# LJacksonPan/RaTrack

Hardware: AMD Instinct MI355X
Metric: radar frame-pairs/sec (backbone forward, eval) at B=64,N=256 per GPU (higher is better)
Workload: dtype f32 (2xfp16 split MFMA: three fp16 products per fp32 product, fp32 accumulate, power-of-two scales per matrix and position); 1 GPU; Track4D.backbone forward, B=64 frame-pairs x N=256 points per GPU, S=512 centroids, eval-mode BN, random-init weights, hipGraph=True, batches in flight=4; global_batch=64, parallelism=replicas x1 (no collective on the forward path)

## Files before the change

include/rtk_fused.h:

```cpp
#ifndef RTK_FUSED_H
#define RTK_FUSED_H

#include "rtk_pointnet2.h"

#ifdef __cplusplus
extern "C" {
#endif

#define RTK_MAX_SRC 4
#define RTK_MAX_LAYERS 4

typedef struct {
    const float *ptr;
    int pitch;
    int channels;
    int per_sample;
} rtk_src_t;

#define RTK_LAYER_SPLIT 0x100
typedef struct {
    const float *w_packed;
    const float *bias;
    int cin16, cout16;
    int act;
    float inv_scale;
} rtk_layer_t;

typedef struct {
    const float *known_feats;
    int pitch, channels, m;
    const int *idx;
    const float *dist2;
    const int *nuniq;
} rtk_interp_t;

RTK_EXPORT int rtk_pointwise_mlp(int rows, int rows_per_sample, const rtk_interp_t *interp, int nsrc,
                                 const rtk_src_t *srcs, const float *sample_bias, int nlayers,
                                 const rtk_layer_t *layers, float *out, int out_pitch, int out_channels,
                                 int out_channel_major, const int *row_nuniq, float *colmax, rtk_stream_t stream);

RTK_EXPORT int rtk_pointwise_mlp_tap(int rows, int rows_per_sample, const rtk_interp_t *interp, const rtk_layer_t *layer, float *out,
                                     int out_pitch, float *colmax, const rtk_layer_t *proj, int frame_split, float *proj_out,
                                     int proj_pitch, rtk_stream_t stream);

RTK_EXPORT int rtk_sa_scale(int samples, int n, int npoint, int nsample, const float *xyz,
                            const float *new_xyz, const int *idx, const float *q, int q_pitch, int c1_16,
                            const float *w1xyz_packed, int nlayers, const rtk_layer_t *layers, float *out,
                            int out_pitch, int out_offset, const int *src_nuniq, const int *dst_nuniq,
                            rtk_stream_t stream);

RTK_EXPORT int rtk_cost_volume(int samples, int n1, int n2, const float *xyz1, const float *xyz2,
                               const int64_t *knn_idx, const float *p1, const float *p2,
                               const float *wd_packed, const rtk_layer_t *layers,
                               const rtk_layer_t *wn, float *out, int out_pitch, rtk_stream_t stream);

RTK_EXPORT int rtk_patch_cost(int samples, int n, const float *xyz, const int64_t *knn_idx,
                              const float *feat, int feat_pitch, const rtk_layer_t *wn, float *out,
                              int out_pitch, int out_channel_major, rtk_stream_t stream);
RTK_EXPORT int rtk_patch_cost_wave16(int samples, int n, const float *xyz, const int64_t *knn_idx,
                                     const float *feat, int feat_pitch, const rtk_layer_t *wn, float *out,
                                     int out_pitch, int out_channel_major, rtk_stream_t stream);

RTK_EXPORT int rtk_pack_split_layer(int cout, int cin, const float *w, int transposed, void *image, float *inv_scale,
                                    rtk_stream_t stream);
RTK_EXPORT int rtk_cost_volume_split(int samples, int n1, int n2, const float *xyz1, const float *xyz2,
                                     const int64_t *knn_idx, const float *p1, const float *p2, const float *wd_packed,
                                     const void *split_images, const float *image_scales, const float *bias2,
                                     const float *bias3, const rtk_layer_t *wn, float *out, int out_pitch, rtk_stream_t stream);
RTK_EXPORT int rtk_cost_volume_split_shared(int samples, int n1, int n2, const float *xyz1, const float *xyz2,
                                            const int64_t *knn_idx, const float *p1, const float *p2, const float *wd_packed,
                                            const void *split_images, const float *image_scales, const float *bias2,
                                            const float *bias3, const rtk_layer_t *wn, float *out, int out_pitch, int workgroups,
                                            rtk_stream_t stream);
RTK_EXPORT int rtk_cost_volume_split_gconst(int samples, int n1, int n2, const float *xyz1, const float *xyz2,
                                            const int64_t *knn_idx, const float *p1, const float *p2, const float *wd_packed,
                                            const void *split_images, const float *image_scales, const float *bias2,
// ... 121 lines not shown
```

ratrack_amd/abi.py:

```python
import ctypes

import torch

_i, _l, _f, _d, _p = ctypes.c_int, ctypes.c_long, ctypes.c_float, ctypes.c_double, ctypes.c_void_p
_ip, _fp, _pp, P = ctypes.POINTER(_i), ctypes.POINTER(_f), ctypes.POINTER(_p), ctypes.POINTER



class Src(ctypes.Structure):
    _fields_ = [("ptr", _p), ("pitch", _i), ("channels", _i), ("per_sample", _i)]


class Layer(ctypes.Structure):
    _fields_ = [("w_packed", _p), ("bias", _p), ("cin16", _i), ("cout16", _i), ("act", _i), ("inv_scale", _f)]


class Interp(ctypes.Structure):
    _fields_ = [("known_feats", _p), ("pitch", _i), ("channels", _i), ("m", _i), ("idx", _p), ("dist2", _p), ("nuniq", _p)]


class GtermJob(ctypes.Structure):
    _fields_ = [("wt", _p), ("bias", _p), ("out", _p), ("cout", _i), ("s0", _i), ("count", _i), ("out_pitch", _i), ("wt2", _p), ("s2", _i)]


# ... 85 lines not shown


class PwWgradJob(ctypes.Structure):
    _fields_ = [("samples", _i), ("positions", _i), ("dz", P(PwOperand)), ("nsrc", _i), ("srcs", P(PwOperand)), ("dw", _p), ("w_pitch", _i),
                ("dbias", _p)]


STRUCTS = {
    "rtk_src_t": Src, "rtk_layer_t": Layer, "rtk_interp_t": Interp, "rtk_gterm_job_t": GtermJob, "rtk_copy_job_t": CopyJob,
    "rtk_layout_job_t": LayoutJob, "rtk_bcn_view_t": View, "rtk_track_frame_t": TrackFrame,
    "rtk_gt_boxes_t": GtBoxes, "rtk_gt_in_t": GtIn, "rtk_gt_out_t": GtOut, "rtk_eval_in_t": EvalIn,
    "rtk_gt_objects_in_t": GtObjectsIn, "rtk_gt_objects_out_t": GtObjectsOut, "rtk_track_score_in_t": ScoreIn,
    "rtk_track_score_state_t": ScoreState, "rtk_track_score_out_t": ScoreOut,
    "rtk_bn_fin_t": BnFin, "rtk_tn_job_t": TnJob, "rtk_pack_job_t": PackJob, "rtk_inverse_index_job_t": InverseIndexJob,
    "rtk_pool_src_t": PoolSrc, "rtk_pw_operand_t": PwOperand, "rtk_pw_wgrad_job_t": PwWgradJob,
}

SIGNATURES = {
    "rtk_furthest_point_sampling": [_i] * 3 + [_p] * 3 + [_p],
    "rtk_gather_points": [_i] * 4 + [_p] * 3 + [_p],
    "rtk_gather_points_grad": [_i] * 4 + [_p] * 3 + [_p],
    "rtk_ball_query": [_i] * 3 + [_f, _i] + [_p] * 3 + [_p],
    "rtk_group_points": [_i] * 5 + [_p] * 3 + [_p],
    "rtk_group_points_grad": [_i] * 5 + [_p] * 3 + [_p],
    "rtk_group_points_grad_set": [_i] * 5 + [_p] * 3 + [_p],
    "rtk_three_nn": [_i] * 3 + [_p] * 4 + [_p],
    "rtk_knn": [_i] * 4 + [_p] * 4 + [_p],
    "rtk_three_interpolate": [_i] * 4 + [_p] * 4 + [_p],
    "rtk_three_interpolate_grad": [_i] * 4 + [_p] * 4 + [_p],
    "rtk_three_interpolate_grad_set": [_i] * 4 + [_p] * 4 + [_p],
    "rtk_knn_point": [_i] * 4 + [_p] * 3 + [_p],
    "rtk_pointwise_mlp": [_i, _i, P(Interp), _i, P(Src), _p, _i, P(Layer), _p, _i, _i, _i, _p, _p, _p],
    "rtk_pointwise_mlp_tap": [_i, _i, P(Interp), P(Layer), _p, _i, _p, P(Layer), _i, _p, _i, _p],
    "rtk_sa_scale": [_i] * 4 + [_p] * 4 + [_i, _i, _p, _i, P(Layer), _p, _i, _i, _p, _p, _p],
    "rtk_cost_volume": [_i] * 3 + [_p] * 6 + [P(Layer), P(Layer), _p, _i, _p],
    "rtk_patch_cost": [_i] * 2 + [_p] * 3 + [_i, P(Layer), _p, _i, _i, _p],
    "rtk_patch_cost_wave16": [_i] * 2 + [_p] * 3 + [_i, P(Layer), _p, _i, _i, _p],
    "rtk_pack_split_layer": [_i, _i, _p, _i, _p, _p, _p],
    "rtk_cost_volume_split": [_i] * 3 + [_p] * 10 + [P(Layer), _p, _i, _p],
    "rtk_cost_volume_split_shared": [_i] * 3 + [_p] * 10 + [P(Layer), _p, _i, _i, _p],
    "rtk_cost_volume_split_gconst": [_i] * 3 + [_p] * 10 + [P(Layer), _p, _i, _i, _p],
    "rtk_cost_volume_split_term": [_i] * 3 + [_p] * 11 + [P(Layer), _p, _i, _i, _p],
    "rtk_sa_scale_split": [_i] * 4 + [_p] * 4 + [_i, _i, _p, _p, _p, _p, _p, _i, _i, _p, _p, _p],
    "rtk_split_mlp2": [_i, _p, _p, _p, _p, _p, _p, _p],
    "rtk_prepare_inputs": [_i] * 2 + [_p] * 6 + [_p],
    "rtk_fps_centroids": [_i] * 3 + [_p] * 8 + [_p],
    "rtk_knn_point_masked": [_i] * 4 + [_p] * 4 + [_p],
    "rtk_fps_relevel": [_i] * 3 + [_p] * 9 + [_i, _p, _p],
    "rtk_gru_step": [_i] * 3 + [_p] * 8 + [_p],
    "rtk_gru_step_head": [_i] * 3 + [_p] * 11 + [_i, _p],
    "rtk_global_terms": [_i, _i, _p, _i, P(GtermJob), _p, _i, _i, _p],
    "rtk_copy_multi": [_i, P(CopyJob), _p],
    "rtk_to_channel_major": [_i] * 3 + [_p, _i, _i, _p, _i, _i, _p],
    "rtk_ball_query_pair": [_i] * 3 + [_f, _i, _f, _i] + [_p] * 5 + [_p],
    "rtk_three_nn_masked": [_i] * 3 + [_p] * 6 + [_p],
    "rtk_geometry_front": [_i] * 4 + [_p, _p, _i] + [_p] * 13 + [_p, _p, _i, _p],
    "rtk_geometry_tables": [_i] * 3 + [_p] * 3 + [_fp, _ip, _pp, _pp, _pp, _p],
    "rtk_to_channel_major_multi": [_i] * 3 + [_p, _p],
    "rtk_log_sinkhorn": [_i, _i, _p, _f, _i, _p, _p],
    "rtk_dbscan": [_i, _p, _i, _p, _p, _f, _d, _i, _p, _p],
    "rtk_dbscan_batched": [_p, _f, _d, _i, _i, _p, _p, _p, _p, _p, _l, _p],
    "rtk_object_descriptors": [_p, _i, _p, _p, _p, _p, _p, _p],
    "rtk_affinity_pairs": [_i, _i] + [_p] * 7 + [_p],
    "rtk_associate_batched": [_i] * 3 + [_p] * 7 + [_f, _i] + [_p] * 9 + [_p],
    "rtk_track_max_objects": [],
    "rtk_gt_labels": [_p, _p, _p],
# ... 70 lines not shown
```

ratrack_amd/csrc/fused_pointwise.hip:

```cpp
#include <string.h>

#include "rtk_common.h"
#include "fused_common.h"
#include "rtk_fused.h"

struct PwParams {
    int rows, rows_per_sample;
    rtk_interp_t interp;
    int nsrc;
    rtk_src_t src[RTK_MAX_SRC];
    const float *sample_bias;
    rtk_layer_t layer[RTK_MAX_LAYERS];
    float *out;
    int out_pitch, out_channels, out_cm;
    const int *row_nuniq;
    float *colmax;
    int gx;
};

template <int V>
__device__ __forceinline__ void init_bias(f4 (&acc)[V], const float *__restrict__ bias, int g) {
#pragma unroll
    for (int v = 0; v < V; ++v) acc[v] = bias_frag(bias, v, g);
}
// ... 247 lines not shown
                    "pointwise_mlp: layer %d expects cin16=%d, got %d (cout16=%d)", l, cin, layers[l].cin16, layers[l].cout16);
        RTK_REQUIRE(((layers[l].act & RTK_LAYER_SPLIT) != 0) == split, "pointwise_mlp: split and fp32 images in one chain (layer %d)", l);
        const size_t prev_floats = l == 0 ? 0 : (split ? (size_t)split16_nf(layers[l - 1].cin16, layers[l - 1].cout16) * 256
                                                        : (size_t)layers[l - 1].cin16 * layers[l - 1].cout16 * 256);
        RTK_REQUIRE(l == 0 || layers[l].w_packed == layers[l - 1].w_packed + prev_floats,
                    "pointwise_mlp: the packed weights of a chain must be contiguous (layer %d)", l);
        P.layer[l] = layers[l];
        P.layer[l].act = layers[l].act & 0xff;
        V[l] = layers[l].cout16;
        cin = V[l];
    }
    P.out = out;
    P.out_pitch = out_pitch;
    P.out_channels = out_channels;
    P.out_cm = out_channel_major;
    P.row_nuniq = row_nuniq;
    P.colmax = colmax;
    RTK_REQUIRE(out_channels > 0 && out_channels <= 16 * cin, "pointwise_mlp: out_channels=%d", out_channels);
    RTK_REQUIRE(out_channel_major || (out_pitch % 4 == 0 && out_pitch >= out_channels), "pointwise_mlp: bad out_pitch %d", out_pitch);
    hipStream_t s = (hipStream_t)stream;
    const bool it = interp != nullptr;
    const long key = ((((long)U * 32 + V[0]) * 32 + V[1]) * 32 + V[2]) * 32 + V[3];
#define PW_CASE(u, v1, v2, v3, v4)                                               \
    case ((((long)(u) * 32 + (v1)) * 32 + (v2)) * 32 + (v3)) * 32 + (v4):        \
        launch_pw<u, v1, v2, v3, v4>(P, it, split, s);                           \
        break;
    switch (key) {
        PW_CASE(1, 2, 0, 0, 0)
        PW_CASE(4, 6, 0, 0, 0)
        PW_CASE(6, 12, 0, 0, 0)
        PW_CASE(8, 4, 0, 0, 0)
        PW_CASE(8, 8, 0, 0, 0)
        PW_CASE(10, 8, 0, 0, 0)
        PW_CASE(8, 16, 0, 0, 0)
        PW_CASE(16, 8, 4, 2, 1)
        PW_CASE(8, 8, 4, 2, 1)
        PW_CASE(25, 2, 0, 0, 0)
        PW_CASE(8, 2, 0, 0, 0)
        default:
            rtk_set_error("pointwise_mlp: no kernel instance for shape U=%d V=(%d,%d,%d,%d)", U, V[0], V[1], V[2], V[3]);
            return RTK_ERR_UNSUPPORTED;
    }
#undef PW_CASE
    RTK_CHECK_LAUNCH("pointwise_mlp");
    return RTK_OK;
}

template <int NW, int F, int NF, int C1, int UP, int VH>
struct WStreamTap {
    static constexpr int NCHUNKS = NF / F, PR = 2 * VH, PH = UP * PR;
    static_assert(NF % F == 0 && PR % F == 0 && C1 < NCHUNKS, "whole chunks; a chunk of the projection is one run of the image");
    const char *blob;
    const char *proj;
    f4 *lds;
    unsigned lane_off;
    int cur, buf, wave, lane;
    __device__ __forceinline__ void issue(int chunk, int into) {
        const char *base;
        if (chunk < C1) {
            base = blob + (size_t)chunk * F * 1024;
        } else {
            const int l = (chunk - C1) * F, h = l / PH, up = (l % PH) / PR, r = l % PR;
            base = proj + (size_t)(PR * (2 * up + h) + r) * 1024;
        }
#pragma unroll
        for (int i = 0; i < (F + NW - 1) / NW; ++i) {
// ... 108 lines not shown
                    (proj[k].act & 0xff) == 0, "pointwise_mlp_tap: projection %d must be a split 128 -> 256 image without activation", k);
    RTK_REQUIRE(out && out_pitch % 4 == 0 && out_pitch >= 128, "pointwise_mlp_tap: bad out_pitch %d", out_pitch);
    TapParams T;
    memset(&T, 0, sizeof(T));
    PwParams &P = T.pw;
    P.rows = rows;
    P.rows_per_sample = rows_per_sample;
    P.interp = *interp;
    P.layer[0] = *layer;
    P.layer[0].act = layer->act & 0xff;
    P.out = out;
    P.out_pitch = out_pitch;
    P.out_channels = 128;
    P.colmax = colmax;
    for (int k = 0; k < 2; ++k) {
        T.proj_w[k] = proj[k].w_packed;
        T.proj_b[k] = proj[k].bias;
        T.proj_inv[k] = proj[k].inv_scale;
    }
    T.frame_split = frame_split;
    T.pout = proj_out;
    T.pout_pitch = proj_pitch;
    const int samples = rows / rows_per_sample;
    const int groups = (rows_per_sample + PW_NW * 16 - 1) / (PW_NW * 16);
    int gx = PW_WGS_TARGET / samples;
    if (gx < 1) gx = 1;
    if (gx > groups) gx = groups;
    P.gx = samples % 8 == 0 ? gx : 0;
    const dim3 blocks = P.gx ? dim3(gx * samples) : dim3(gx, samples);
    pointwise_tap_kernel<8, 8, 16><<<blocks, 64 * PW_NW, 0, (hipStream_t)stream>>>(T);
    RTK_CHECK_LAUNCH("pointwise_mlp_tap");
    return RTK_OK;
}
```

ratrack_amd/fused.py:

```python
import ctypes
import os
import types

import torch

from . import _lib
from . import pointnet2_hip as _native
from .abi import CopyJob as _CopyJob, GtermJob as _GtJob, Interp as _Interp, Layer as _Layer, Src as _Src, stream as _stream

ACT_NONE, ACT_RELU, ACT_LEAKY, ACT_SIGMOID = 0, 1, 2, 3


def copy_multi(pairs):
    for i in range(0, len(pairs), 8):
        part = pairs[i:i + 8]
        jobs = (_CopyJob * len(part))()
        for j, (d, s_) in enumerate(part):
            assert d.is_contiguous() and s_.is_contiguous() and d.shape == s_.shape and d.dtype == s_.dtype and d.device == s_.device
            jobs[j].src, jobs[j].dst, jobs[j].bytes = s_.data_ptr(), d.data_ptr(), d.numel() * d.element_size()
        _lib.call("rtk_copy_multi", len(part), jobs, _stream())


def ceil16(c):
    return (c + 15) // 16 * 16
# ... 99 lines not shown
    p = split2_f16(wp, scale).reshape(2, V, 16, U2, 2, 4, 4)
    return p.permute(3, 1, 0, 5, 2, 4, 6).contiguous().reshape(-1), inv


PW_SPLIT = True
LAYER_SPLIT = 0x100


def pad_bias(b, cout):
    out = torch.zeros(ceil16(cout), dtype=torch.float32, device=b.device)
    out[:b.numel()] = b.float()
    return out


class Chain:

    def split_arr(self):
        if self._split is None:
            packed = [pack_layer_split16(w.to(self._device)) for w, _ in self._layers]
            blob = torch.cat([im for im, _ in packed]).contiguous()
            arr = (_Layer * len(self._layers))()
            off = boff = 0
            for i, (w, act) in enumerate(self._layers):
                cout, cin = w.shape
                u, v = ceil16(cin) // 16, ceil16(cout) // 16
                arr[i].w_packed = blob.data_ptr() + 2 * off
                arr[i].bias = self.bias.data_ptr() + 4 * boff
                arr[i].cin16, arr[i].cout16, arr[i].act, arr[i].inv_scale = u, v, act | LAYER_SPLIT, packed[i][1]
                off += ((u + 1) // 2) * v * 2 * 512
                boff += v * 16
            self._split = (arr, blob)
        return self._split[0]

    def __init__(self, layers, device):
        packs, biases, meta = [], [], []
        self.dims = [tuple(w.shape) for w, _, _ in layers]
        for w, b, act in layers:
            cout, cin = w.shape
            packs.append(pack_layer(w.to(device)))
            biases.append(pad_bias(b.to(device), cout))
            meta.append((ceil16(cin) // 16, ceil16(cout) // 16, act))
        self.blob = torch.cat(packs).contiguous()
        self.bias = torch.cat(biases).contiguous()
        self._layers, self._device, self._split = [(w, act) for w, _, act in layers], device, None
        arr = (_Layer * len(layers))()
        woff = boff = 0
        for i, (u, v, act) in enumerate(meta):
            arr[i].w_packed = self.blob.data_ptr() + 4 * woff
            arr[i].bias = self.bias.data_ptr() + 4 * boff
            arr[i].cin16, arr[i].cout16, arr[i].act = u, v, act
            woff += u * v * 256
            boff += v * 16
        self.arr = arr
        self.n = len(layers)
        self.cout = layers[-1][0].shape[0]
        self.cout16 = meta[-1][1]


def _colptr(t, col=0):
    assert t.dim() == 2 and t.stride(1) == 1 and t.dtype == torch.float32
    return t.data_ptr() + 4 * col, t.stride(0)


def pointwise(rows, rows_per_sample, srcs, chain, out, out_channels=None, sample_bias=None, interp=None, channel_major=False,
              row_nuniq=None, colmax=None):
    arr = (_Src * max(len(srcs), 1))()
    for i, (t, ch, per) in enumerate(srcs):
        ptr, pitch = _colptr(t)
        arr[i].ptr, arr[i].pitch, arr[i].channels, arr[i].per_sample = ptr, pitch, ch, int(per)
    ip = None
    if interp is not None:
        kf, ch, m, idx, d2 = interp[:5]
        nu = interp[5] if len(interp) > 5 else None
        ptr, pitch = _colptr(kf)
        ip = ctypes.pointer(_Interp(ptr, pitch, ch, m, idx.data_ptr(), d2.data_ptr(), nu.data_ptr() if nu is not None else None))
    oc = out_channels if out_channels is not None else chain.cout
    if _TRACE is not None:
        macs = sum(co * ci for co, ci in chain.dims) + (3 * interp[1] if interp is not None else 0)
        _TRACE.append(("pointwise", _live_rows(row_nuniq, rows_per_sample, rows // rows_per_sample), macs))
    if channel_major:
        optr, opitch = out.data_ptr(), 0
    else:
        optr, opitch = _colptr(out)
    _lib.call("rtk_pointwise_mlp", rows, rows_per_sample, ip, len(srcs), arr,
              sample_bias.data_ptr() if sample_bias is not None else None, chain.n, chain.split_arr() if PW_SPLIT else chain.arr, optr, opitch, oc,
              int(channel_major), row_nuniq.data_ptr() if row_nuniq is not None else None,
              colmax.data_ptr() if colmax is not None else None, _stream())
    return out


pointwise_mlp = pointwise


def pointwise_tap(rows, rows_per_sample, chain, out, colmax, interp, proj, frame_split, proj_out):
    assert PW_SPLIT and chain.n == 1 and all(c.n == 1 for c in proj)
    kf, ch, m, idx, d2 = interp[:5]
    nu = interp[5] if len(interp) > 5 else None
    ptr, pitch = _colptr(kf)
    ip = ctypes.pointer(_Interp(ptr, pitch, ch, m, idx.data_ptr(), d2.data_ptr(), nu.data_ptr() if nu is not None else None))
    if _TRACE is not None:
        _TRACE.append(("pointwise", rows, sum(co * ci for co, ci in chain.dims) + 3 * ch))
        _TRACE.append(("pointwise", rows, sum(co * ci for co, ci in proj[0].dims)))
    pa = (_Layer * 2)(proj[0].split_arr()[0], proj[1].split_arr()[0])
    optr, opitch = _colptr(out)
    pptr, ppitch = _colptr(proj_out)
    _lib.call("rtk_pointwise_mlp_tap", rows, rows_per_sample, ip, chain.split_arr(), optr, opitch, colmax.data_ptr(), pa, frame_split,
              pptr, ppitch, _stream())
    return out, proj_out


def offset_image(w4, device):
    cout = w4.shape[0]
    V = ceil16(cout) // 16
    wp = torch.zeros(V * 16, 4, dtype=torch.float32, device=device)
    wp[:cout] = w4.float().to(device)
    return wp.reshape(V, 16, 4).permute(0, 2, 1).contiguous().reshape(-1)


class _WeightNet:

    def __init__(self, sd, prefix, device):
        g = lambda k: sd[prefix + k].double()
        wa, ba = g(".mlp_convs.0.weight").reshape(8, 3), g(".mlp_convs.0.bias")
        wb, bb = g(".mlp_convs.1.weight").reshape(8, 8), g(".mlp_convs.1.bias")
        wc, bc = g(".mlp_convs.2.weight").reshape(-1, 8), g(".mlp_convs.2.bias")
        self.wa = offset_image(torch.cat([wa, ba[:, None]], 1), device)
        self.wb, self.bb = pack_layer(wb.to(device)), pad_bias(bb.to(device), 8)
        self.wc, self.bc = pack_layer(wc.to(device)), pad_bias(bc.to(device), wc.shape[0])
        arr = (_Layer * 3)()
        arr[0].w_packed, arr[0].cin16, arr[0].cout16 = self.wa.data_ptr(), 1, 1
        arr[1].w_packed, arr[1].bias, arr[1].cin16, arr[1].cout16 = self.wb.data_ptr(), self.bb.data_ptr(), 1, 1
        arr[2].w_packed, arr[2].bias, arr[2].cin16, arr[2].cout16 = self.wc.data_ptr(), self.bc.data_ptr(), 1, ceil16(wc.shape[0]) // 16
        self.arr = arr


SA_SPLIT = True


class _SAScale:

    def __init__(self, sd, prefix, nsample, radius, device):
        self.nsample, self.radius = nsample, float(radius)
        ws = []
# ... 9 lines not shown
        self.cout = ws[-1][0].shape[0]
        self.split_image = None
        if SA_SPLIT and len(ws) == 2 and self.cout == 64 and self.c1 in (32, 64) and nsample in (16, 32) and torch.device(device).type == "cuda":
            w2 = ws[1][0].float().to(device).contiguous()
            self.split_bias = ws[1][1].float().to(device).contiguous()
            self.split_image, self.split_scale = pack_split_device(w2)
            torch.cuda.current_stream().synchronize()


class _PNHeadWeights:

    RADII = [[2, 4], [4, 8], [8, 16]]
    NSAMPLES = [[4, 8], [8, 16], [16, 32]]

    def __init__(self, sd, prefix, device):
        d = lambda k: sd[prefix + k].double()
        self.scales = [[_SAScale(sd, "%ssa%d.mlps.%d" % (prefix, l + 1, s), self.NSAMPLES[l][s], self.RADII[l][s], device)
                        for s in range(2)] for l in range(3)]
        self.wq1 = torch.cat([self.scales[0][0].wf, self.scales[0][1].wf], 0)
        self.trans = []
        for l in (1, 2):
            wl, bl = d("linear%d.weight" % l), d("linear%d.bias" % l)
            rows, bias = [wl], [bl]
            for s in range(2):
                wf = self.scales[l][s].wf
                rows.append(wf @ wl)
                bias.append(wf @ bl)
            self.trans.append(Chain([(torch.cat(rows, 0), torch.cat(bias, 0), ACT_NONE)], device))
        self.lin3 = Chain([(d("linear3.weight"), d("linear3.bias"), ACT_NONE)], device)
        self.fp = {}
        for name in ("fp3", "fp2", "fp1"):
            w, b = fold_bn(sd[prefix + name + ".mlp.layer0.conv.weight"], prefix + name + ".mlp.layer0.bn.bn", sd)
            self.fp[name] = Chain([(w, b, ACT_RELU)], device)


FUSED_GEOMETRY = True
GEOMETRY_POISON = None
CHECK_FPS_RELEVEL = False

INTERP_LEVELS = (("fp3", 2, 3), ("fp2", 1, 2), ("fp1", 0, 1))


def check_fps_relevel(xyz1, idx, new_xyz, nuniq):
    S_, npoint, _ = xyz1.shape
    src = xyz1
    for l in range(idx.shape[0]):
        i = torch.empty(S_, npoint, dtype=torch.int32, device=src.device)
        out = torch.empty(S_, npoint, 3, dtype=torch.float32, device=src.device)
        cnt = torch.empty(S_, dtype=torch.int32, device=src.device)
        _lib.call("rtk_fps_centroids", S_, npoint, npoint, src.data_ptr(), i.data_ptr(), out.data_ptr(), cnt.data_ptr(), None, None, None, None,
                  _stream())
        assert torch.equal(i, idx[l].view(S_, npoint)), "fps_relevel: level %d indices differ from the full selection" % (l + 2)
        assert torch.equal(out, new_xyz[l].view(S_, npoint, 3)), "fps_relevel: level %d centroids differ" % (l + 2)
        assert torch.equal(cnt, nuniq[l].view(-1)), "fps_relevel: level %d exhausted-cloud counters differ" % (l + 2)
        src = out


def _geometry_workspace(xyz, npoint, knn_frames, finite, zeros, fused_geo):
    (S_, n, _), dev = xyz.shape, xyz.device
    ball_sizes = [S_ * npoint * ns for row in _PNHeadWeights.NSAMPLES for ns in row]
    nn_sizes = [S_ * (n if u == 0 else npoint) * 3 for _, u, _ in INTERP_LEVELS]
    sizes = [S_ * npoint] * 3 + [S_] * 3 + [S_, 2 * S_, S_] + ball_sizes + nn_sizes
    unfilled = fused_geo and not finite and zeros is None
    alloc = zeros or (lambda n_, dtype, device: torch.zeros(n_, dtype=dtype, device=device))
    if unfilled:
        ints = torch.empty(sum(sizes), dtype=torch.int32, device=dev)
        if GEOMETRY_POISON is not None:
            ints.fill_(GEOMETRY_POISON)
# ... 191 lines not shown
    if _TRACE is not None:
        macs = sc.nsample * (4 * sc.c1 + sum(co * ci for co, ci in sc.chain.dims))
        _TRACE.append(("sa_scale", _live_rows(geo.nuniq[lvl], geo.npoint, geo.samples), macs))
    if sc.split_image is not None:
        _lib.call("rtk_sa_scale_split", geo.samples, src.shape[1], geo.npoint, sc.nsample, src.data_ptr(), dst.data_ptr(),
                  geo.ball[lvl][s].data_ptr(), qptr, qpitch, sc.c1, sc.w1img.data_ptr(), sc.split_image.data_ptr(), sc.split_scale.data_ptr(),
                  sc.split_bias.data_ptr(),
                  optr, opitch, out_offset, src_nu, geo.nuniq[lvl].data_ptr(), _stream())
        return
    _lib.call("rtk_sa_scale", geo.samples, src.shape[1], geo.npoint, sc.nsample, src.data_ptr(), dst.data_ptr(),
              geo.ball[lvl][s].data_ptr(), qptr, qpitch, ceil16(sc.c1) // 16, sc.w1img.data_ptr(),
              sc.chain.n, sc.chain.arr, optr, opitch, out_offset, src_nu, geo.nuniq[lvl].data_ptr(), _stream())


def run_pnhead(W, geo, q1, out=None, gmax=None, tap=None):
    S_, n, S = geo.samples, geo.n, geo.npoint
    dev = q1.device
    new = lambda rows, c: torch.empty(rows, c, dtype=torch.float32, device=dev)
    nu = geo.nuniq
    sa1 = new(S_ * S, 64)
    geo.wait(0)
    sa_scale(geo, W, 0, 0, q1, 0, sa1, 0)
    sa_scale(geo, W, 0, 1, q1, 16, sa1, 32)
    t1 = pointwise(S_ * S, S, [(sa1, 64, False)], W.trans[0], new(S_ * S, 96), row_nuniq=nu[0])
    sa2 = new(S_ * S, 96)
    geo.wait(1)
    sa_scale(geo, W, 1, 0, t1, 32, sa2, 0)
    sa_scale(geo, W, 1, 1, t1, 64, sa2, 32)
    t2 = pointwise(S_ * S, S, [(sa2, 96, False)], W.trans[1], new(S_ * S, 192), row_nuniq=nu[1])
    sa3 = new(S_ * S, 128)
    geo.wait(2)
    sa_scale(geo, W, 2, 0, t2, 64, sa3, 0)
    sa_scale(geo, W, 2, 1, t2, 128, sa3, 64)
    l3 = pointwise(S_ * S, S, [(sa3, 128, False)], W.lin3, new(S_ * S, 64), row_nuniq=nu[2])
    geo.wait("nn")
    d2, idx, m = geo.nn["fp3"]
    f3 = pointwise(S_ * S, S, [(t2[:, 0:64], 64, False)], W.fp["fp3"], new(S_ * S, 128), row_nuniq=nu[1],
                   interp=(l3, 64, m, idx.reshape(-1, 3), d2.reshape(-1, 3), nu[2]))
    d2, idx, m = geo.nn["fp2"]
    f2 = pointwise(S_ * S, S, [(t1[:, 0:32], 32, False)], W.fp["fp2"], new(S_ * S, 128), row_nuniq=nu[0],
                   interp=(f3, 128, m, idx.reshape(-1, 3), d2.reshape(-1, 3), nu[1]))
    d2, idx, m = geo.nn["fp1"]
    if gmax is None:
        gmax = torch.zeros(S_, 128, dtype=torch.float32, device=dev)
    out = out if out is not None else new(S_ * n, 128)
    interp = (f2, 128, m, idx.reshape(-1, 3), d2.reshape(-1, 3), nu[0])
    if tap is not None:
        pointwise_tap(S_ * n, n, W.fp["fp1"], out, gmax, interp, *tap)
    else:
        pointwise(S_ * n, n, [], W.fp["fp1"], out, interp=interp, colmax=gmax)
    return out, gmax


class FusedBackbone:

    def __init__(self, model, split=True):
        sd = {k: v.detach() for k, v in model.state_dict().items()}
        dev = next(model.parameters()).device
        self.dev = dev
        self.npoint = model.pn_head.sa1.npoint
        g = lambda k: torch.stack([sd["fd_layer.torchGRU.%s_l%d" % (k, l)].float() for l in range(5)])
        self.gru_wih = g("weight_ih").transpose(1, 2).contiguous()
        self.gru_whh = g("weight_hh").transpose(1, 2).contiguous()
        self.gru_bih, self.gru_bhh = g("bias_ih").contiguous(), g("bias_hh").contiguous()
        self.kernel_events = None
        self.kernel_token = None
        self._split_hook = None
        self.side, self.use_side_stream = None, True
        self.cv_shared = False
        self.proj_tap = True
        self._last_cv = None
        self.enc = _PNHeadWeights(sd, "pn_head.", dev)
        self.dec = _PNHeadWeights(sd, "fd_layer.mse.", dev)
        z = lambda n: torch.zeros(n, dtype=torch.float64, device=sd["bin_score"].device)
        self.enc_q1 = Chain([(self.enc.wq1, z(32), ACT_NONE)], dev)
        self.enc_q1_w = self.enc.wq1.float().to(dev).contiguous()
        w0 = sd["fc_layer.mlp_convs.0.weight"].double().reshape(256, 515)
        b0 = sd["fc_layer.mlp_convs.0.bias"].double()
        self.p1_loc = Chain([(w0[:, 0:128], z(256), ACT_NONE)], dev)
        self.p2_loc = Chain([(w0[:, 256:384], z(256), ACT_NONE)], dev)
        tr = lambda w: w.float().t().contiguous().to(dev)
        self.p1_glob_wt, self.p1_glob_b = tr(w0[:, 128:256]), b0.float().to(dev).contiguous()
        self.p2_glob_wt = tr(w0[:, 384:512])
        self.cv_wd = offset_image(torch.cat([w0[:, 512:515], z(256)[:, None]], 1), dev)
        self.cv_layers = Chain([(sd["fc_layer.mlp_convs.%d.weight" % i].double().reshape(256, 256),
                                 sd["fc_layer.mlp_convs.%d.bias" % i].double(), ACT_LEAKY) for i in (1, 2)], dev)
        self.cv_split = bool(split)
        w23 = [sd["fc_layer.mlp_convs.%d.weight" % i].double().reshape(256, 256).float().to(dev).contiguous() for i in (1, 2)]
        self.cv_bias23 = torch.stack([sd["fc_layer.mlp_convs.%d.bias" % i].double().float() for i in (1, 2)]).to(dev).contiguous()
        self.cv_images = torch.empty(2 * SPLIT_IMAGE_256, dtype=torch.int16, device=dev)
        self.cv_scales = torch.empty(2, dtype=torch.float32, device=dev)
        for l, w in enumerate(w23):
            _lib.call("rtk_pack_split_layer", 256, 256, w.data_ptr(), 0, self.cv_images[l * SPLIT_IMAGE_256:].data_ptr(),
                      self.cv_scales[l:].data_ptr(), _stream())
        torch.cuda.current_stream().synchronize()
        self.wn1 = _WeightNet(sd, "fc_layer.weightnet1", dev)
        self.wn2 = _WeightNet(sd, "fc_layer.weightnet2", dev)
        def predictor(prefix, first_cols):
            layers = []
            for i in range(3):
                w, b = fold_bn(sd["%s.sf_mlp.%d.0.weight" % (prefix, i)], "%s.sf_mlp.%d.1" % (prefix, i), sd)
                layers.append([w, b, ACT_RELU])
            return layers
# ... 46 lines not shown
            global_terms(glob, [(self.p1_glob_wt, self.p1_glob_b, st, 0, self.p2_glob_wt, B), (self.dec_q1_glob_wt, None, sbq, 0)],
                         bcast=feat12[:, 128:], n=N)
            p1, p2 = p12[:B * N], p12[B * N:]
        else:
            st = None
            sb1, sb2 = new(B, 256), new(B, 256)
            global_terms(glob, [(self.p1_glob_wt, self.p1_glob_b, sb1, 0), (self.p2_glob_wt, None, sb2, B), (self.dec_q1_glob_wt, None, sbq, 0)],
                         bcast=feat12[:, 128:], n=N)
            p1 = pointwise(B * N, N, [(f1, 128, False)], self.p1_loc, new(B * N, 256), sample_bias=sb1)
            p2 = pointwise(B * N, N, [(f2, 128, False)], self.p2_loc, new(B * N, 256), sample_bias=sb2)
        x1, x2 = xyz[:B], xyz[B:]
        geo.wait("knn")
        knn1, knn2 = geo.knn
        cor1 = new(B * N, 256)
        self._last_cv = (B, N, x1, x2, knn1, p1, p2, cor1, st)
        if self._split_hook is not None:
            geo.events.clear()
            self._split_hook()
        else:
            ev = self.kernel_events
            if ev is not None:
                e0, e1 = torch.cuda.Event(enable_timing=True), torch.cuda.Event(enable_timing=True)
                e0.record()
            self._cost_volume(*self._last_cv)
            if ev is not None:
                e1.record()
                ev.append((e0, e1))
        cor = new(B * N, 256)
        if _TRACE is not None:
            _TRACE.append(("patch_cost", B * N * 16, (3 * 8 + 8 * 8 + 8 * 256) + 256))
        _lib.call("rtk_patch_cost", B, N, x1.data_ptr(), knn2.data_ptr(), cor1.data_ptr(), 256, self.wn2.arr, cor.data_ptr(), 256, 0,
                  _stream())
        cls = torch.empty(B, N, dtype=torch.float32, device=dev)
        pointwise(B * N, N, [(cor, 256, False)], self.cls_head, cls, out_channels=1, channel_major=True)
        q1d = pointwise(B * N, N, [(raw[:B * N], 2, False), (f1, 128, False), (cor, 256, False)], self.dec_q1, new(B * N, 32),
                        sample_bias=sbq)
        prop, gfeat = run_pnhead(self.dec, geo.head(B), q1d, gmax=gmax[2 * B:])
        if h is None:
            h = torch.zeros(5, B, 128, device=dev, dtype=torch.float32)
        gout, h_out, sbf = self._gru_step(gfeat, h)
        flow = torch.empty(B, 3, N, dtype=torch.float32, device=dev)
        pointwise(B * N, N, [(prop, 128, False)], self.flow_head, flow, out_channels=3, sample_bias=sbf, channel_major=True)
        f12 = feat12.view(2 * B, N, 256).permute(0, 2, 1)
        pc1_features, pc2_features = f12[:B], f12[B:]
        cor_cm = cor.view(B, N, 256).permute(0, 2, 1)
        prop_cm = prop.view(B, N, 128).permute(0, 2, 1)
        return flow, h_out, cls, cor_cm, pc1_features, pc2_features, prop_cm

    def _cost_volume(self, B, N, x1, x2, knn1, p1, p2, cor1, sample_term=None):
        assert sample_term is None or self.cv_split
        if _TRACE is not None:
            _TRACE.append(("cost_volume", B * N * 16, 3 * 256 + 2 * 256 * 256 + (3 * 8 + 8 * 8 + 8 * 256) + 256))
        if self.cv_split:
            step = B if B * N <= CV_SPLIT_MAX_ROWS else max(1, CV_SPLIT_MAX_ROWS // N)
            for b0 in range(0, B, step):
                nb = min(step, B - b0)
                wgs = cv_shared_workgroups(nb, N, x1.device) if self.cv_shared else 0
                r0 = b0 * N
                if sample_term is not None:
                    _lib.call("rtk_cost_volume_split_term", nb, N, N, x1[b0:].data_ptr(), x2[b0:].data_ptr(), knn1[b0:].data_ptr(),
                              p1[r0:].data_ptr(), p2[r0:].data_ptr(), sample_term[b0:].data_ptr(), self.cv_wd.data_ptr(),
                              self.cv_images.data_ptr(), self.cv_scales.data_ptr(), self.cv_bias23[0].data_ptr(), self.cv_bias23[1].data_ptr(),
                              self.wn1.arr, cor1[r0:].data_ptr(), 256, wgs, _stream())
                    continue
                _lib.call("rtk_cost_volume_split_shared", nb, N, N, x1[b0:].data_ptr(), x2[b0:].data_ptr(), knn1[b0:].data_ptr(), p1[r0:].data_ptr(),
                          p2[r0:].data_ptr(), self.cv_wd.data_ptr(), self.cv_images.data_ptr(), self.cv_scales.data_ptr(),
                          self.cv_bias23[0].data_ptr(), self.cv_bias23[1].data_ptr(), self.wn1.arr, cor1[r0:].data_ptr(), 256, wgs, _stream())
            return
        _lib.call("rtk_cost_volume", B, N, N, x1.data_ptr(), x2.data_ptr(), knn1.data_ptr(), p1.data_ptr(), p2.data_ptr(),
# ... 169 lines not shown
```

Measured before the change: 110,400 frame-pairs/s.

## Fuse cls head with decoder q1 pointwise pass; fold linear3 into fp3 interpolation

Adds a pair kernel that reads the shared decoder inputs (raw, f1, cor) once and computes both the decoder q1 projection and the 4-layer classification head, which uses cor as its only input. This removes one launch and a second read of the 256-channel cor rows. Separately, the lin3 layer is folded algebraically into the fp3 first layer, so fp3 interpolates the raw sa3 features directly and the lin3 pointwise pass is skipped. The trade-off is more registers per thread in the pair kernel and 128-channel interpolation in place of 64-channel, plus the fold's exactness relies on linear3 having no activation.

```diff
diff --git a/include/rtk_fused.h b/include/rtk_fused.h
--- a/include/rtk_fused.h
+++ b/include/rtk_fused.h
@@ -42,6 +42,10 @@
 RTK_EXPORT int rtk_pointwise_mlp_tap(int rows, int rows_per_sample, const rtk_interp_t *interp, const rtk_layer_t *layer, float *out,
                                      int out_pitch, float *colmax, const rtk_layer_t *proj, int frame_split, float *proj_out,
                                      int proj_pitch, rtk_stream_t stream);
+
+RTK_EXPORT int rtk_pointwise_mlp_pair(int rows, int rows_per_sample, int nsrc, const rtk_src_t *srcs, const float *sample_bias,
+                                      const rtk_layer_t *layer_a, float *out_a, int out_a_pitch, int out_a_channels, int nlayers_b,
+                                      const rtk_layer_t *layers_b, float *out_b, int out_b_channels, rtk_stream_t stream);
 
 RTK_EXPORT int rtk_sa_scale(int samples, int n, int npoint, int nsample, const float *xyz,
                             const float *new_xyz, const int *idx, const float *q, int q_pitch, int c1_16,
diff --git a/ratrack_amd/abi.py b/ratrack_amd/abi.py
--- a/ratrack_amd/abi.py
+++ b/ratrack_amd/abi.py
@@ -141,6 +141,7 @@
     "rtk_knn_point": [_i] * 4 + [_p] * 3 + [_p],
     "rtk_pointwise_mlp": [_i, _i, P(Interp), _i, P(Src), _p, _i, P(Layer), _p, _i, _i, _i, _p, _p, _p],
     "rtk_pointwise_mlp_tap": [_i, _i, P(Interp), P(Layer), _p, _i, _p, P(Layer), _i, _p, _i, _p],
+    "rtk_pointwise_mlp_pair": [_i, _i, _i, P(Src), _p, P(Layer), _p, _i, _i, _i, P(Layer), _p, _i, _p],
     "rtk_sa_scale": [_i] * 4 + [_p] * 4 + [_i, _i, _p, _i, P(Layer), _p, _i, _i, _p, _p, _p],
     "rtk_cost_volume": [_i] * 3 + [_p] * 6 + [P(Layer), P(Layer), _p, _i, _p],
     "rtk_patch_cost": [_i] * 2 + [_p] * 3 + [_i, P(Layer), _p, _i, _i, _p],
diff --git a/ratrack_amd/csrc/fused_pointwise.hip b/ratrack_amd/csrc/fused_pointwise.hip
--- a/ratrack_amd/csrc/fused_pointwise.hip
+++ b/ratrack_amd/csrc/fused_pointwise.hip
@@ -303,6 +303,7 @@
         PW_CASE(8, 4, 0, 0, 0)
         PW_CASE(8, 8, 0, 0, 0)
         PW_CASE(10, 8, 0, 0, 0)
+        PW_CASE(12, 8, 0, 0, 0)
         PW_CASE(8, 16, 0, 0, 0)
         PW_CASE(16, 8, 4, 2, 1)
         PW_CASE(8, 8, 4, 2, 1)
@@ -477,3 +478,138 @@
     RTK_CHECK_LAUNCH("pointwise_mlp_tap");
     return RTK_OK;
 }
+
+struct PairParams {
+    PwParams pw;
+    rtk_layer_t lb[4];
+    float *out_b;
+    int out_b_channels;
+};
+
+template <int U, int VA, int UB, int V1, int V2, int V3, int V4>
+__global__ __launch_bounds__(64 * PW_NW, 2) void pointwise_pair_kernel(const PairParams T) {
+    __shared__ __attribute__((aligned(16))) f4 s_w[2 * PW_F * 64];
+    const PwParams &P = T.pw;
+    const int lane = threadIdx.x & 63, g = lane >> 4, j = lane & 15;
+    const int wave_in_wg = threadIdx.x >> 6;
+    int b, bx, nbx;
+    rtk_decode_block(P.gx, b, bx, nbx);
+    const int rps = P.rows_per_sample;
+    const int groups = (rps + PW_NW * 16 - 1) / (PW_NW * 16);
+    if (bx >= groups) return;
+    constexpr int FA = split16_nf(U, VA), F1 = split16_nf(UB, V1), F2 = split16_nf(V1, V2), F3 = split16_nf(V2, V3), F4 = split16_nf(V3, V4);
+    WStream<PW_NW, PW_F, FA + F1 + F2 + F3 + F4> ws;
+    ws.start_deferred(reinterpret_cast<const f4 *>(P.layer[0].w_packed), s_w, wave_in_wg, lane);
+
+    int ustart[RTK_MAX_SRC + 1];
+    ustart[0] = 0;
+#pragma unroll
+    for (int s = 0; s < RTK_MAX_SRC; ++s) ustart[s + 1] = ustart[s] + (s < P.nsrc ? (P.src[s].channels + 15) >> 4 : 0);
+    const int uend = ustart[RTK_MAX_SRC];
+
+    for (int G = bx; G < groups; G += nbx) {
+        asm volatile("" ::: "memory");
+        const int r = G * (PW_NW * 16) + wave_in_wg * 16 + j;
+        const bool valid = r < rps;
+        const int p = b * rps + (valid ? r : rps - 1);
+        f4 h[U];
+        const float *rowp[RTK_MAX_SRC];
+        const float *dummy = reinterpret_cast<const float *>(P.layer[0].w_packed);
+#pragma unroll
+        for (int q = 0; q < RTK_MAX_SRC; ++q)
+            rowp[q] = q < P.nsrc ? P.src[q].ptr + (P.src[q].per_sample ? (size_t)b : (size_t)p) * P.src[q].pitch + 4 * g : nullptr;
+#pragma unroll
+        for (int u = 0; u < U; ++u) {
+            const float *rp = rowp[0];
+            int us = ustart[0], ch = P.src[0].channels;
+#pragma unroll
+            for (int q = 1; q < RTK_MAX_SRC; ++q)
+                if (q < P.nsrc && u >= ustart[q]) { rp = rowp[q]; us = ustart[q]; ch = P.src[q].channels; }
+            const int c = 16 * (u - us);
+            const bool ok = u < uend && c + 4 * g < ch;
+            const f4 v = *reinterpret_cast<const f4 *>(ok ? rp + c : dummy);
+            h[u] = ok ? v : f4_zero();
+        }
+        {
+            f4 a[VA];
+            pw_layer<true, U, VA, 0>(ws, h, a, P.layer[0], g, P.sample_bias ? P.sample_bias + (size_t)b * 16 * VA : nullptr, true);
+            store_tile<VA>(P, a, p, b, g, valid);
+        }
+        f4 hb[UB];
+#pragma unroll
+        for (int u = 0; u < UB; ++u) hb[u] = h[U - UB + u];
+        f4 a1[V1], a2[V2], a3[V3], a4[V4];
+        pw_layer<true, UB, V1, FA>(ws, hb, a1, T.lb[0], g, nullptr, false);
+        pw_layer<true, V1, V2, FA + F1>(ws, a1, a2, T.lb[1], g, nullptr, false);
+        pw_layer<true, V2, V3, FA + F1 + F2>(ws, a2, a3, T.lb[2], g, nullptr, false);
+        pw_layer<true, V3, V4, FA + F1 + F2 + F3>(ws, a3, a4, T.lb[3], g, nullptr, false);
+        if (valid) {
+            float *o = T.out_b + (size_t)b * T.out_b_channels * rps + (p - b * rps);
+#pragma unroll
+            for (int v = 0; v < V4; ++v) {
+                const int c = 16 * v + 4 * g;
+                if (c + 0 < T.out_b_channels) o[(size_t)(c + 0) * rps] = a4[v].x;
+                if (c + 1 < T.out_b_channels) o[(size_t)(c + 1) * rps] = a4[v].y;
+                if (c + 2 < T.out_b_channels) o[(size_t)(c + 2) * rps] = a4[v].z;
+                if (c + 3 < T.out_b_channels) o[(size_t)(c + 3) * rps] = a4[v].w;
+            }
+        }
+    }
+    ws.finish();
+}
+
+extern "C" int rtk_pointwise_mlp_pair(int rows, int rows_per_sample, int nsrc, const rtk_src_t *srcs, const float *sample_bias,
+                                      const rtk_layer_t *layer_a, float *out_a, int out_a_pitch, int out_a_channels, int nlayers_b,
+                                      const rtk_layer_t *layers_b, float *out_b, int out_b_channels, rtk_stream_t stream) {
+    RTK_REQUIRE(rows > 0 && rows_per_sample > 0 && rows % rows_per_sample == 0 && rows / rows_per_sample <= 65535,
+                "pointwise_mlp_pair: bad row counts (%d, %d)", rows, rows_per_sample);
+    RTK_REQUIRE(nsrc >= 1 && nsrc <= RTK_MAX_SRC && srcs && layer_a && layers_b && out_a && out_b, "pointwise_mlp_pair: nsrc=%d", nsrc);
+    PairParams T;
+    memset(&T, 0, sizeof(T));
+    PwParams &P = T.pw;
+    P.rows = rows;
+    P.rows_per_sample = rows_per_sample;
+    P.nsrc = nsrc;
+    int U = 0;
+    for (int s = 0; s < nsrc; ++s) {
+        RTK_REQUIRE(srcs[s].ptr && srcs[s].pitch % 4 == 0 && srcs[s].channels > 0 && srcs[s].pitch >= ((srcs[s].channels + 3) / 4) * 4,
+                    "pointwise_mlp_pair: bad source %d (pitch %d, channels %d)", s, srcs[s].pitch, srcs[s].channels);
+        P.src[s] = srcs[s];
+        U += (srcs[s].channels + 15) / 16;
+    }
+    const int UB = (srcs[nsrc - 1].channels + 15) / 16;
+    RTK_REQUIRE(U == 25 && UB == 16 && nlayers_b == 4, "pointwise_mlp_pair: no kernel instance for U=%d UB=%d, %d layers", U, UB, nlayers_b);
+    RTK_REQUIRE(layer_a->w_packed && layer_a->bias && (layer_a->act & RTK_LAYER_SPLIT) && layer_a->cin16 == 25 && layer_a->cout16 == 2,
+                "pointwise_mlp_pair: chain A must be one split 25 -> 2 block layer");
+    static const int vb[5] = {16, 8, 4, 2, 1};
+    const float *w = layer_a->w_packed + (size_t)split16_nf(25, 2) * 256;
+    for (int l = 0; l < 4; ++l) {
+        RTK_REQUIRE(layers_b[l].bias && (layers_b[l].act & RTK_LAYER_SPLIT) && layers_b[l].cin16 == vb[l] && layers_b[l].cout16 == vb[l + 1],
+                    "pointwise_mlp_pair: chain B layer %d must be a split %d -> %d block layer", l, vb[l], vb[l + 1]);
+        RTK_REQUIRE(layers_b[l].w_packed == w, "pointwise_mlp_pair: the images must be contiguous, chain A's first (chain B layer %d)", l);
+        w += (size_t)split16_nf(vb[l], vb[l + 1]) * 256;
+        T.lb[l] = layers_b[l];
+        T.lb[l].act = layers_b[l].act & 0xff;
+    }
+    P.layer[0] = *layer_a;
+    P.layer[0].act = layer_a->act & 0xff;
+    P.sample_bias = sample_bias;
+    P.out = out_a;
+    P.out_pitch = out_a_pitch;
+    P.out_channels = out_a_channels;
+    RTK_REQUIRE(out_a_channels > 0 && out_a_channels <= 32 && out_a_pitch % 4 == 0 && out_a_pitch >= out_a_channels,
+                "pointwise_mlp_pair: bad output A (%d channels, pitch %d)", out_a_channels, out_a_pitch);
+    RTK_REQUIRE(out_b_channels > 0 && out_b_channels <= 16, "pointwise_mlp_pair: out_b_channels=%d", out_b_channels);
+    T.out_b = out_b;
+    T.out_b_channels = out_b_channels;
+    const int samples = rows / rows_per_sample;
+    const int groups = (rows_per_sample + PW_NW * 16 - 1) / (PW_NW * 16);
+    int gx = PW_WGS_TARGET / samples;
+    if (gx < 1) gx = 1;
+    if (gx > groups) gx = groups;
+    P.gx = samples % 8 == 0 ? gx : 0;
+    const dim3 blocks = P.gx ? dim3(gx * samples) : dim3(gx, samples);
+    pointwise_pair_kernel<25, 2, 16, 8, 4, 2, 1><<<blocks, 64 * PW_NW, 0, (hipStream_t)stream>>>(T);
+    RTK_CHECK_LAUNCH("pointwise_mlp_pair");
+    return RTK_OK;
+}
diff --git a/ratrack_amd/fused.py b/ratrack_amd/fused.py
--- a/ratrack_amd/fused.py
+++ b/ratrack_amd/fused.py
@@ -155,6 +155,22 @@
             self._split = (arr, blob)
         return self._split[0]
 
+    def split_pair(self, other):
+        got = self._pairs.get(id(other))
+        if got is None:
+            mine, theirs = self.split_arr(), other.split_arr()
+            blob = torch.cat([self._split[1], other._split[1]]).contiguous()
+            arrs, off = [], 0
+            for src in (mine, theirs):
+                arr = (_Layer * len(src))()
+                for i, l in enumerate(src):
+                    arr[i].w_packed, arr[i].bias = blob.data_ptr() + 2 * off, l.bias
+                    arr[i].cin16, arr[i].cout16, arr[i].act, arr[i].inv_scale = l.cin16, l.cout16, l.act, l.inv_scale
+                    off += ((l.cin16 + 1) // 2) * l.cout16 * 2 * 512
+                arrs.append(arr)
+            got = self._pairs[id(other)] = (arrs[0], arrs[1], blob, other)
+        return got[0], got[1]
+
     def __init__(self, layers, device):
         packs, biases, meta = [], [], []
         self.dims = [tuple(w.shape) for w, _, _ in layers]
@@ -166,6 +182,7 @@
         self.blob = torch.cat(packs).contiguous()
         self.bias = torch.cat(biases).contiguous()
         self._layers, self._device, self._split = [(w, act) for w, _, act in layers], device, None
+        self._pairs = {}
         arr = (_Layer * len(layers))()
         woff = boff = 0
         for i, (u, v, act) in enumerate(meta):
@@ -232,6 +249,22 @@
     return out, proj_out
 
 
+def pointwise_pair(rows, rows_per_sample, srcs, chain_a, out_a, sample_bias, chain_b, out_b, out_b_channels):
+    assert PW_SPLIT and chain_a.n == 1 and chain_b.n == 4
+    arr = (_Src * len(srcs))()
+    for i, (t, ch, per) in enumerate(srcs):
+        ptr, pitch = _colptr(t)
+        arr[i].ptr, arr[i].pitch, arr[i].channels, arr[i].per_sample = ptr, pitch, ch, int(per)
+    if _TRACE is not None:
+        _TRACE.append(("pointwise", rows, sum(co * ci for co, ci in chain_b.dims)))
+        _TRACE.append(("pointwise", rows, sum(co * ci for co, ci in chain_a.dims)))
+    la, lb = chain_a.split_pair(chain_b)
+    optr, opitch = _colptr(out_a)
+    _lib.call("rtk_pointwise_mlp_pair", rows, rows_per_sample, len(srcs), arr, sample_bias.data_ptr() if sample_bias is not None else None,
+              la, optr, opitch, chain_a.cout, chain_b.n, lb, out_b.data_ptr(), out_b_channels, _stream())
+    return out_a, out_b
+
+
 def offset_image(w4, device):
     cout = w4.shape[0]
     V = ceil16(cout) // 16
@@ -307,8 +340,12 @@
         for name in ("fp3", "fp2", "fp1"):
             w, b = fold_bn(sd[prefix + name + ".mlp.layer0.conv.weight"], prefix + name + ".mlp.layer0.bn.bn", sd)
             self.fp[name] = Chain([(w, b, ACT_RELU)], device)
-
-
+            if name == "fp3":
+                wl, bl = d("linear3.weight"), d("linear3.bias")
+                self.fp3c = Chain([(torch.cat([w[:, :64] @ wl, w[:, 64:]], 1), b + w[:, :64] @ bl, ACT_RELU)], device)
+
+
+FOLD_LIN3 = True
 FUSED_GEOMETRY = True
 GEOMETRY_POISON = None
 CHECK_FPS_RELEVEL = False
@@ -566,11 +603,13 @@
     geo.wait(2)
     sa_scale(geo, W, 2, 0, t2, 64, sa3, 0)
     sa_scale(geo, W, 2, 1, t2, 128, sa3, 64)
-    l3 = pointwise(S_ * S, S, [(sa3, 128, False)], W.lin3, new(S_ * S, 64), row_nuniq=nu[2])
+    if not FOLD_LIN3:
+        l3 = pointwise(S_ * S, S, [(sa3, 128, False)], W.lin3, new(S_ * S, 64), row_nuniq=nu[2])
     geo.wait("nn")
     d2, idx, m = geo.nn["fp3"]
-    f3 = pointwise(S_ * S, S, [(t2[:, 0:64], 64, False)], W.fp["fp3"], new(S_ * S, 128), row_nuniq=nu[1],
-                   interp=(l3, 64, m, idx.reshape(-1, 3), d2.reshape(-1, 3), nu[2]))
+    known, known_ch, chain = (sa3, 128, W.fp3c) if FOLD_LIN3 else (l3, 64, W.fp["fp3"])
+    f3 = pointwise(S_ * S, S, [(t2[:, 0:64], 64, False)], chain, new(S_ * S, 128), row_nuniq=nu[1],
+                   interp=(known, known_ch, m, idx.reshape(-1, 3), d2.reshape(-1, 3), nu[2]))
     d2, idx, m = geo.nn["fp2"]
     f2 = pointwise(S_ * S, S, [(t1[:, 0:32], 32, False)], W.fp["fp2"], new(S_ * S, 128), row_nuniq=nu[0],
                    interp=(f3, 128, m, idx.reshape(-1, 3), d2.reshape(-1, 3), nu[1]))
@@ -603,6 +642,7 @@
         self.side, self.use_side_stream = None, True
         self.cv_shared = False
         self.proj_tap = True
+        self.pair_readers = True
         self._last_cv = None
         self.enc = _PNHeadWeights(sd, "pn_head.", dev)
         self.dec = _PNHeadWeights(sd, "fd_layer.mse.", dev)
@@ -715,9 +755,12 @@
         _lib.call("rtk_patch_cost", B, N, x1.data_ptr(), knn2.data_ptr(), cor1.data_ptr(), 256, self.wn2.arr, cor.data_ptr(), 256, 0,
                   _stream())
         cls = torch.empty(B, N, dtype=torch.float32, device=dev)
-        pointwise(B * N, N, [(cor, 256, False)], self.cls_head, cls, out_channels=1, channel_major=True)
-        q1d = pointwise(B * N, N, [(raw[:B * N], 2, False), (f1, 128, False), (cor, 256, False)], self.dec_q1, new(B * N, 32),
-                        sample_bias=sbq)
+        dsrc = [(raw[:B * N], 2, False), (f1, 128, False), (cor, 256, False)]
+        if self.pair_readers and PW_SPLIT:
+            q1d, _ = pointwise_pair(B * N, N, dsrc, self.dec_q1, new(B * N, 32), sbq, self.cls_head, cls, 1)
+        else:
+            pointwise(B * N, N, [(cor, 256, False)], self.cls_head, cls, out_channels=1, channel_major=True)
+            q1d = pointwise(B * N, N, dsrc, self.dec_q1, new(B * N, 32), sample_bias=sbq)
         prop, gfeat = run_pnhead(self.dec, geo.head(B), q1d, gmax=gmax[2 * B:])
         if h is None:
             h = torch.zeros(5, B, 128, device=dev, dtype=torch.float32)
```

After: 111,700 frame-pairs/s, median of 6. 1.01x the previous value.
